# WU-CVGL/CasualHDRSplat

Measured on AMD Instinct MI355X. Metric: train-step images/sec (fwd+bwd raster) @ 1M Gaussians 1080p, higher is better.
Workload: dtype f32; 1 GPU; c3: 1000000 Gaussians, 1920x1080, SH degree 3, HDR radiance + CRF tone-map, 1 pose(s)/view, 1 view(s)/step (one per GPU); num_rendered_R=6777809, R_prime=3025699, pixel_pair_evals_E=559372855, seed=0, binning=sync-free fixed capacity 1.25*R, launch=eager (one enqueue per kernel)

## Files before the change

### casualhdrsplat_amd/csrc/hs_common.h

```cpp
#pragma once
#include <hip/hip_runtime.h>
#include <stdint.h>

#include "../../include/hdrsplat.h"

#if defined(__HIP_DEVICE_COMPILE__) && !defined(__gfx950__)
#error "libhdrsplat is written for gfx950 (MI355X) only: build with --offload-arch=gfx950"
#endif

namespace hs {

void set_error(const char* fmt, ...);

#define HS_HIP_CHECK(expr)                                                                         \
    do {                                                                                           \
        hipError_t e_ = (expr);                                                                    \
        if (e_ != hipSuccess) {                                                                    \
            ::hs::set_error("%s failed: %s (%s:%d)", #expr, hipGetErrorString(e_), __FILE__, __LINE__); \
            return HS_EHIP;                                                                        \
        }                                                                                          \
    } while (0)
#define HS_LAUNCH_CHECK() HS_HIP_CHECK(hipGetLastError())

#ifndef HS_TUNE_CRF_IN_RENDER_TAIL
#define HS_TUNE_CRF_IN_RENDER_TAIL 1
#endif

#ifndef HS_TUNE_COUNT_SORT
#define HS_TUNE_COUNT_SORT 1
#endif

constexpr int kTile = HS_TILE;
constexpr int kRecF4 = 4;
constexpr int kPairF4 = 4;
constexpr int kInstF4 = 4;
constexpr int kRecFloats = 4 * kRecF4;
constexpr int kPairFloats = 4 * kPairF4;
constexpr int kInstFloats = 4 * kInstF4;
constexpr int kSortBlock = 256;
constexpr int kDepthBins = 512, kDepthDigitBits = 9;
#ifndef HS_TUNE_DEPTH_ITEMS
#define HS_TUNE_DEPTH_ITEMS 8
#endif
constexpr int kDepthSortItems = HS_TUNE_DEPTH_ITEMS, kDepthSortLook = 8;
constexpr int kPairSortItems = 16, kPairSortLook = 8;
constexpr int kU64SortItems = 16;
constexpr int kDepthTile = kDepthSortItems * kDepthBins, kPairTile = kPairSortItems * kSortBlock, kU64Tile = kU64SortItems * kSortBlock;
static_assert(kPairTile == kU64Tile && kDepthTile >= kPairTile, "the scratch of every sort is sized for the smallest tile");
constexpr int kSortTileMin = kPairTile;

static inline int64_t align_up(int64_t v, int64_t a) { return (v + a - 1) / a * a; }
static inline int ceil_div(int64_t a, int64_t b) { return (int)((a + b - 1) / b); }

static inline int tile_bits(uint32_t n) {
    int b = 0;
    while (n) { ++b; n >>= 1; }
    return b;
}

int launch_preprocess_fwd(const hs_fwd_args& a, const hs_layout& L, hipStream_t s, uint32_t frame_tag);
int launch_scan(const hs_fwd_args& a, const hs_layout& L, hipStream_t s);
int launch_cov3d(const hs_fwd_args& a, const hs_layout& L, hipStream_t s);
int launch_binning(const hs_fwd_args& a, const hs_layout& L, hipStream_t s, uint32_t frame_tag);
int launch_empty_frame(hs_counters* clear, uint2* ranges, int64_t ntiles, uint32_t* counters_host, const hs_counters* counters,
                       hipStream_t s);
int launch_render_fwd(const hs_fwd_args& a, const hs_layout& L, hipStream_t s, unsigned long long* stats = nullptr);
int launch_render_bwd(const hs_bwd_args& a, const hs_layout& L, hipStream_t s, unsigned long long* stats = nullptr,
                      unsigned long long* timeline = nullptr, bool crf_in_tail = false);
int render_stats_count();
struct CrfReduce;
int launch_crf_bwd(const hs_bwd_args& a, const hs_layout& L, hipStream_t s, CrfReduce* defer, bool in_render_tail = false);
int launch_preprocess_bwd(const hs_bwd_args& a, const hs_layout& L, hipStream_t s, bool segsum, bool project,
                          const CrfReduce* crf_reduce);
int launch_mark_visible(int P, const float* means3D, const float* view, uint8_t* vis, hipStream_t s);
int launch_spline_poses(int J, int T, int kind, const float* delta, const float* base, const float* times, float* w2c,
                        float* jac, int* seg, hipStream_t s);
int launch_sh_backward_views(int P, int M, int deg, int V, const float* means3D, const float* camposes,
                             const float* view_colors, float* d_shs, hipStream_t s);

constexpr int kGhistCopies = 16;
constexpr int kGhistWords = kGhistCopies * 8 * 256;
constexpr int kTicketWords = 128, kDepthBitsAt = 32, kDepthBitsCopies = 16, kDepthBitsWords = 4 * kDepthBitsCopies;
static_assert(kDepthBitsAt >= 8 && kDepthBitsAt % 2 == 0 && kDepthBitsAt + kDepthBitsWords <= kTicketWords, "depth bits live in the ticket row");
__host__ __device__ inline int64_t sweep_pass_words(int64_t nblk, int bins = 256) { return nblk * bins; }
static inline int64_t sort_scratch_words(int64_t n, int passes, int tile, int bins = 256) {
    return n > 0 ? kGhistWords + kTicketWords + (int64_t)passes * sweep_pass_words((n + tile - 1) / tile, bins) : 0;
}
static inline int64_t depth_scratch_words(int64_t I) { return sort_scratch_words(I, 4, kDepthTile, kDepthBins); }
int64_t sort_tmp_bytes(int64_t n);
constexpr int kMsdBits = 12, kMsdBuckets = 1 << kMsdBits;
#ifndef HS_TUNE_MSD_RANGE
// ... 226 lines not shown
```

### casualhdrsplat_amd/csrc/preprocess.hip

```cpp
#include "hs_common.h"


namespace hs {

namespace {

__device__ constexpr float SH_C0 = 0.28209479177387814f;
__device__ constexpr float SH_C1 = 0.4886025119029199f;
__device__ constexpr float SH_C2[5] = {1.0925484305920792f, -1.0925484305920792f, 0.31539156525252005f,
                                       -1.0925484305920792f, 0.5462742152960396f};
__device__ constexpr float SH_C3[7] = {-0.5900435899266435f, 2.890611442640554f, -0.4570457994644658f,
                                       0.3731763325901154f,  -0.4570457994644658f, 1.445305721320277f,
                                       -0.5900435899266435f};

struct Ewa {
    float tx, ty, tz;
    bool clamp_x, clamp_y;
    float a0[3], a1[3];
    float fx, fy;
};

__device__ __forceinline__ void quat_to_R(const float* q, float* R) {
    float r = q[0], x = q[1], y = q[2], z = q[3];
    R[0] = 1.f - 2.f * (y * y + z * z); R[1] = 2.f * (x * y - r * z);       R[2] = 2.f * (x * z + r * y);
// ... 94 lines not shown
            g[14][0] = SH_C3[5] * 2.f * x * z; g[14][1] = SH_C3[5] * -2.f * y * z; g[14][2] = SH_C3[5] * (xx - yy);
            g[15][0] = SH_C3[6] * (3.f * xx - 3.f * yy); g[15][1] = SH_C3[6] * -6.f * x * y;
        }
    }
}

struct PreFwd {
    int P, M, W, H, N;
    float tanfovx, tanfovy, mod;
    const float* view; const float* proj; const float* campos;
    const float* means; const float* opac; const float* shs; const float* colors; const float* scales;
    const float* rots; const float* cov_pre;
    float4* rec; float* depth; int* radii_inst; uint32_t* tiles; float* cov3D; uint8_t* clamped;
    uint2* binfo;
    int* radii_out;
    uint2* depth_pairs; hs_counters* counters; uint2* ranges; int64_t n_vtiles;
    uint32_t* sort_zero; int64_t n_sort_zero;
    int64_t bits_at;
    uint32_t frame_tag;
    uint32_t* pair_zero; int64_t n_pair_zero;
    bool antialias;
    int act;
};

#ifndef HS_TUNE_PF_REC_LDS
#define HS_TUNE_PF_REC_LDS 1
#endif
#ifndef HS_TUNE_PF_EARLY
#define HS_TUNE_PF_EARLY 1
#endif
#ifndef HS_TUNE_PF_WAVES
#define HS_TUNE_PF_WAVES 5
#endif
#if HS_TUNE_PF_WAVES > 0
#define HS_PF_OCC __attribute__((amdgpu_waves_per_eu(HS_TUNE_PF_WAVES, HS_TUNE_PF_WAVES)))
#else
#define HS_PF_OCC
#endif
template <int DEG>
__global__ void __launch_bounds__(256) HS_PF_OCC preprocess_fwd_kernel(PreFwd p) {
    __shared__ uint32_t s_two[2];
    if (p.depth_pairs) {
        if (threadIdx.x < 2) s_two[threadIdx.x] = 0u;
        __syncthreads();
    }
    uint32_t depth_key = 0xFFFFFFFFu;
    const int64_t lin = (int64_t)blockIdx.x * 256 + threadIdx.x;
    const int xcd = blockIdx.x & 7, seq = blockIdx.x >> 3;
    const int pose = seq % p.N;
    const int64_t g64 = ((int64_t)(seq / p.N) * 8 + xcd) * 256 + threadIdx.x;
    uint32_t ntiles = 0;
#if HS_TUNE_PF_REC_LDS
    __shared__ float4 s_rec[4][64 * 4];
    float4 rec_a = make_float4(0.f, 0.f, 0.f, 0.f), rec_b = rec_a, rec_c = rec_a;
#endif
    if (g64 < (int64_t)p.P) {
    const int g = (int)g64;
    const int64_t idx = (int64_t)pose * p.P + g;
    const float* V = p.view + 16 * pose;
    const float* PM = p.proj + 16 * pose;

    int my_radius = 0;
    uint2 bi = make_uint2(0u, 0u);
    float4 ra = make_float4(0.f, 0.f, 0.f, 0.f), rb = ra, rc = ra;
    float depth = 0.f;
    uint8_t clampbits = 0;

    const float x = p.means[3 * g], y = p.means[3 * g + 1], z = p.means[3 * g + 2];
    float sc[3] = {0.f, 0.f, 0.f};
    float4 q4 = make_float4(0.f, 0.f, 0.f, 0.f);
    float s6[6] = {0.f, 0.f, 0.f, 0.f, 0.f, 0.f};
    if (p.cov_pre) {
#pragma unroll
        for (int k = 0; k < 6; ++k) s6[k] = p.cov_pre[6 * g + k];
    } else {
        sc[0] = p.scales[3 * g]; sc[1] = p.scales[3 * g + 1]; sc[2] = p.scales[3 * g + 2];
        q4 = reinterpret_cast<const float4*>(p.rots)[g];
    }
    const float opac_in = p.opac[g];
    const float pvx = xform_row(V, 0, x, y, z), pvy = xform_row(V, 1, x, y, z), pvz = xform_row(V, 2, x, y, z);
    const float phx = xform_row(PM, 0, x, y, z), phy = xform_row(PM, 1, x, y, z), phw = xform_row(PM, 3, x, y, z);
    const float pw = 1.0f / (phw + 0.0000001f);
    const float ppx = phx * pw, ppy = phy * pw;
    constexpr int NCF = (DEG + 1) * (DEG + 1);
    float shr[3 * NCF];
#pragma unroll
    for (int k = 0; k < 3 * NCF; ++k) shr[k] = 0.f;
    bool have_sh = false;
    bool vis = false;
#if HS_TUNE_PF_EARLY
    const bool early = !p.colors && pvz > 0.2f && fabsf(ppx) < 1.5f && fabsf(ppy) < 1.5f;
    if (early) {
        const float* sh = p.shs + (int64_t)g * p.M * 3;
#pragma unroll
        for (int k = 0; k < 3 * NCF; ++k) shr[k] = sh[k];
        have_sh = true;
    }
#endif
    if (!p.cov_pre && (pose == 0 || pvz > 0.2f)) {
        float q[4] = {q4.x, q4.y, q4.z, q4.w};
        cov3d_from_scale_rot(sc, p.mod, q, s6);
    }

    if (pvz > 0.2f) {

        Ewa e;
        ewa_setup(V, p.W, p.H, p.tanfovx, p.tanfovy, pvx, pvy, pvz, e);
        float u0[3], u1[3];
        sym_mul(s6, e.a0, u0);
        sym_mul(s6, e.a1, u1);
        const float ca = dot3(e.a0, u0) + 0.3f;
        const float cb = dot3(e.a1, u0);
        const float cc = dot3(e.a1, u1) + 0.3f;
        const float det = ca * cc - cb * cb;
        if (det != 0.0f) {
            const float det_inv = 1.f / det;
            const float conA = cc * det_inv, conB = -cb * det_inv, conC = ca * det_inv;
            const float mid = 0.5f * (ca + cc);
            const float disc = sqrtf(fmaxf(0.1f, mid * mid - det));
            const float lam1 = mid + disc, lam2 = mid - disc;
            const int rad = (int)ceilf(3.f * sqrtf(fmaxf(lam1, lam2)));
            const float pix_x = ((ppx + 1.0f) * (float)p.W - 1.0f) * 0.5f;
            const float pix_y = ((ppy + 1.0f) * (float)p.H - 1.0f) * 0.5f;
            const int gx = (p.W + kTile - 1) / kTile, gy = (p.H + kTile - 1) / kTile;
            const int rminx = min(gx, max(0, (int)((pix_x - (float)rad) / (float)kTile)));
            const int rminy = min(gy, max(0, (int)((pix_y - (float)rad) / (float)kTile)));
            const int rmaxx = min(gx, max(0, (int)((pix_x + (float)rad + (float)(kTile - 1)) / (float)kTile)));
            const int rmaxy = min(gy, max(0, (int)((pix_y + (float)rad + (float)(kTile - 1)) / (float)kTile)));
            const int area = (rmaxx - rminx) * (rmaxy - rminy);
            if (area != 0) {
                vis = true;
                my_radius = rad;
                ntiles = (uint32_t)area;
                bi = make_uint2((uint32_t)rminx | ((uint32_t)rminy << 16),
                                (uint32_t)(rmaxx - rminx) | ((uint32_t)(rmaxy - rminy) << 16));
                depth = pvz;
                ra = make_float4(pix_x, pix_y, conA, conB);
                float opac = opac_in;
                if (p.antialias) {
                    const float det0 = (ca - 0.3f) * (cc - 0.3f) - cb * cb;
                    opac = opac * sqrtf(fmaxf(0.000025f, det0 / det));
                }
                rb = make_float4(conC, opac, 0.f, 0.f);
                rc = make_float4(0.f, pvz, __int_as_float(rad), 0.f);
            }
        }
    }
    if (vis) {
        float col[3];
        if (p.colors) {
            col[0] = p.colors[3 * g]; col[1] = p.colors[3 * g + 1]; col[2] = p.colors[3 * g + 2];
        } else {
            const float* cp = p.campos + 3 * pose;
            const float dx = x - cp[0], dy = y - cp[1], dz = z - cp[2];
            const float len = sqrtf((dx * dx + dy * dy) + dz * dz);
            const float ux = dx / len, uy = dy / len, uz = dz / len;
            float b[(DEG + 1) * (DEG + 1)];
            sh_basis<DEG>(ux, uy, uz, b);
            if (!have_sh) {
                const float* sh = p.shs + (int64_t)g * p.M * 3;
#pragma unroll
                for (int k = 0; k < 3 * NCF; ++k) shr[k] = sh[k];
            }
            float acc[3] = {b[0] * shr[0], b[0] * shr[1], b[0] * shr[2]};
#pragma unroll
            for (int k = 1; k < (DEG + 1) * (DEG + 1); ++k) {
                acc[0] = acc[0] + b[k] * shr[3 * k + 0];
                acc[1] = acc[1] + b[k] * shr[3 * k + 1];
                acc[2] = acc[2] + b[k] * shr[3 * k + 2];
            }
#pragma unroll
            for (int ch = 0; ch < 3; ++ch) {
                if (p.act == 1) {
                    col[ch] = expf(acc[ch]);
                } else if (p.act == 2) {
                    col[ch] = acc[ch] > 20.f ? acc[ch] : log1pf(expf(acc[ch]));
                } else {
                    float v = acc[ch] + 0.5f;
                    if (v < 0.f) clampbits |= (uint8_t)(1u << ch);
                    col[ch] = fmaxf(v, 0.f);
                }
            }
        }
        rb.z = col[0]; rb.w = col[1]; rc.x = col[2];
    }
#if HS_TUNE_PF_REC_LDS
    rec_a = ra; rec_b = rb; rec_c = rc;
#else
    p.rec[kRecF4 * idx + 0] = ra;
    p.rec[kRecF4 * idx + 1] = rb;
    p.rec[kRecF4 * idx + 2] = rc;
    p.rec[kRecF4 * idx + 3] = make_float4(0.f, 0.f, 0.f, 0.f);
#endif
    p.depth[idx] = depth;
    p.radii_inst[idx] = my_radius;
    p.tiles[idx] = ntiles;
    p.binfo[idx] = bi;
    p.clamped[idx] = clampbits;
    if (p.N == 1) p.radii_out[g] = my_radius;
    else if (my_radius > 0) atomicMax(p.radii_out + g, my_radius);
    if (p.depth_pairs) {
        if (my_radius > 0) depth_key = __float_as_uint(depth);
        p.depth_pairs[idx] = make_uint2(depth_key, (uint32_t)idx);
    }
    }
#if HS_TUNE_PF_REC_LDS
    {
        const int lane = threadIdx.x & 63, wave = threadIdx.x >> 6;
        float4* w = s_rec[wave];
        const int sw = (lane >> 2) & 3;
        w[lane * 4 + (0 ^ sw)] = rec_a;
        w[lane * 4 + (1 ^ sw)] = rec_b;
        w[lane * 4 + (2 ^ sw)] = rec_c;
        w[lane * 4 + (3 ^ sw)] = make_float4(0.f, 0.f, 0.f, 0.f);
        __builtin_amdgcn_fence(__ATOMIC_RELEASE, "wavefront");
        __builtin_amdgcn_wave_barrier();
        const int64_t g_w0 = g64 - lane;
        const int nvalid = (int)min((int64_t)64, (int64_t)p.P - g_w0);
        float4* dst = p.rec + kRecF4 * ((int64_t)pose * p.P + g_w0);
#pragma unroll
        for (int j = 0; j < 4; ++j) {
            const int f = j * 64 + lane, r = f >> 2, k = f & 3;
            if (r < nvalid) dst[f] = w[r * 4 + (k ^ ((r >> 2) & 3))];
        }
    }
#endif
    if (p.depth_pairs) {
        depth_bits_accumulate(depth_key, depth_key != 0xFFFFFFFFu,
                              reinterpret_cast<unsigned long long*>(p.sort_zero + p.bits_at), p.frame_tag, s_two);
        for (int64_t t = lin; t < p.n_vtiles; t += (int64_t)gridDim.x * 256) p.ranges[t] = make_uint2(0u, 0u);
        for (int64_t t = lin; t < p.n_sort_zero; t += (int64_t)gridDim.x * 256)
            if (t < p.bits_at || t >= p.bits_at + kDepthBitsWords) p.sort_zero[t] = 0u;
        for (int64_t t = lin; t < p.n_pair_zero; t += (int64_t)gridDim.x * 256) p.pair_zero[t] = 0u;
        if (lin == 0) {
            p.counters->overflow = 0u;
            p.counters->reserved[1] = (uint32_t)((int64_t)p.P * p.N);
            p.counters->reserved[2] = 0u; p.counters->reserved[3] = 0u;
            p.counters->reserved[4] = 0u;
        }
    }
}

__global__ void __launch_bounds__(256) cov3d_kernel(int P, float mod, const float* scales, const float* rots, const float* cov_pre,
                                                    float* cov3D) {
    const int g = blockIdx.x * 256 + threadIdx.x;
    if (g >= P) return;
    float s6[6];
    if (cov_pre) {
#pragma unroll
        for (int k = 0; k < 6; ++k) s6[k] = cov_pre[6 * (int64_t)g + k];
    } else {
        float sc[3] = {scales[3 * g], scales[3 * g + 1], scales[3 * g + 2]};
        const float4 q4 = reinterpret_cast<const float4*>(rots)[g];
        float q[4] = {q4.x, q4.y, q4.z, q4.w};
        cov3d_from_scale_rot(sc, mod, q, s6);
    }
#pragma unroll
    for (int k = 0; k < 6; ++k) cov3D[6 * (int64_t)g + k] = s6[k];
}

__global__ void mark_visible_kernel(int P, const float* means, const float* V, uint8_t* vis) {
    int i = blockIdx.x * 256 + threadIdx.x;
    if (i >= P) return;
    vis[i] = xform_row(V, 2, means[3 * i], means[3 * i + 1], means[3 * i + 2]) > 0.2f;
}

__global__ void __launch_bounds__(256) pair_segsum_kernel(SegsumArgs sg, CrfReduce crf_reduce) {
// ... 639 lines not shown
```

### casualhdrsplat_amd/csrc/render.hip

```cpp
#include "hs_common.h"

namespace hs {

namespace {

constexpr float kAlphaMin = 1.0f / 255.0f;
constexpr float kAlphaMax = 0.99f;
constexpr float kTmin = 0.0001f;
constexpr float kLogEps = 1e-8f;


enum {
    kStBwdTrips = 0,
    kStBwdEmpty = 1,
    kStBwdActivePix = 2,
    kStBwdCulled = 3,
    kStBwdHist = 4,
    kStBwdStaged = 10,
    kStBwdBatches = 11,
    kStFwdTrips = 12, kStFwdEmpty = 13, kStFwdActivePix = 14, kStFwdCulled = 15, kStFwdStaged = 16, kStFwdBatches = 17,
    kStCount = 24
};
struct WaveStats {
    unsigned long long v[kStCount];
    __device__ __forceinline__ void clear() {
#pragma unroll
        for (int i = 0; i < kStCount; ++i) v[i] = 0;
    }
    __device__ __forceinline__ void flush(unsigned long long* dst) const {
        if ((threadIdx.x & 63) == 0) {
#pragma unroll
            for (int i = 0; i < kStCount; ++i)
                if (v[i]) atomicAdd(dst + i, v[i]);
        }
    }
};

template <int CTRL, int ROW_MASK = 0xF>
__device__ __forceinline__ float dpp(float v) {
    return __int_as_float(__builtin_amdgcn_update_dpp(0, __float_as_int(v), CTRL, ROW_MASK, 0xF, false));
}
__device__ __forceinline__ float wave_sum_hi(float v) {
    v += dpp<0xB1>(v);
    v += dpp<0x4E>(v);
    v += dpp<0x141>(v);
    v += dpp<0x140>(v);
    v += dpp<0x142, 0xA>(v);
    v += dpp<0x143, 0xC>(v);
    return v;
}
__device__ __forceinline__ float halve16(float x, float y) {
    auto r = __builtin_amdgcn_permlane16_swap(__float_as_uint(x), __float_as_uint(y), false, false);
    return __uint_as_float(r[0]) + __uint_as_float(r[1]);
}
template <bool TEN>
__device__ __forceinline__ void reduce_in_rows(const float* g, float g9, float& w0, float& w1, float& w2) {
    float z0, z1, z2, z3, z4;
    if constexpr (TEN) {
        asm("s_nop 1\n\t"
// ... 49 lines not shown
template <bool TEN>
__device__ __forceinline__ void group_reduce(const float* g, float g9, int xor16_addr, float& t0, float& t1) {
    float w0, w1, w2;
    reduce_in_rows<TEN>(g, g9, w0, w1, w2);
    const float u0 = halve16(w0, w1);
    const float u1 = w2 + __int_as_float(__builtin_amdgcn_ds_bpermute(xor16_addr, __float_as_int(w2)));
    t0 = reduce_in_quads(u0);
    t1 = reduce_in_quads(u1);
}

__device__ __forceinline__ int mask_prefix(uint64_t m) {
    return (int)__builtin_amdgcn_mbcnt_hi((uint32_t)(m >> 32), __builtin_amdgcn_mbcnt_lo((uint32_t)m, 0u));
}

__device__ __forceinline__ uint32_t wave_max_u32(uint32_t v) {
#pragma unroll
    for (int d = 32; d >= 1; d >>= 1) v = max(v, (uint32_t)__shfl_xor((int)v, d));
    return v;
}

struct Crf {
    const float* table;
    int K;
    float umin, umax, dt;
};

__device__ __forceinline__ void crf_locate(const Crf& c, float Hv, int& i, float& f, float& xv, bool& interior) {
    xv = Hv * c.dt;
    const float u = __logf(fmaxf(xv, kLogEps));
    float s = (u - c.umin) / (c.umax - c.umin) * (float)(c.K - 1);
    bool in = true;
    if (!(s > 0.f)) { s = 0.f; in = false; }
    if (s >= (float)(c.K - 1)) { s = (float)(c.K - 1); in = false; }
    i = (int)floorf(s);
    if (i > c.K - 2) i = c.K - 2;
    f = s - (float)i;
    interior = in && (xv > kLogEps);
}
__device__ __forceinline__ float crf_eval(const Crf& c, int ch, float Hv) {
    int i; float f, xv; bool in;
    crf_locate(c, Hv, i, f, xv, in);
    const float* t = c.table + ch * c.K;
    return t[i] * (1.f - f) + t[i + 1] * f;
}
__device__ __forceinline__ float crf_grad_H(const Crf& c, int ch, float Hv, float g) {
    int i; float f, xv; bool in;
    crf_locate(c, Hv, i, f, xv, in);
    if (!in) return 0.f;
    const float* t = c.table + ch * c.K;
    const float scale = (float)(c.K - 1) / (c.umax - c.umin);
    return g * (t[i + 1] - t[i]) * scale / xv * c.dt;
}

constexpr float kLog2e = 1.4426950408889634f;

typedef float f2 __attribute__((ext_vector_type(2)));

#ifndef HS_NO_OPSEL_ASM
__device__ __forceinline__ f2 pk_fma_hi(f2 pair, f2 w, f2 acc) {
    asm("v_pk_fma_f32 %0, %1, %2, %0 op_sel:[1,0,0] op_sel_hi:[1,1,1]" : "+v"(acc) : "v"(pair), "v"(w));
    return acc;
}
__device__ __forceinline__ f2 pk_mul_hi(f2 pair, f2 w) {
    f2 r;
    asm("v_pk_mul_f32 %0, %1, %2 op_sel:[1,0] op_sel_hi:[1,1]" : "=v"(r) : "v"(pair), "v"(w));
    return r;
}
#else
__device__ __forceinline__ f2 pk_fma_hi(f2 pair, f2 w, f2 acc) { return acc + f2{pair.y, pair.y} * w; }
__device__ __forceinline__ f2 pk_mul_hi(f2 pair, f2 w) { return f2{pair.y, pair.y} * w; }
#endif

__device__ __forceinline__ void scale_entry(float4& a, float4& b) {
    a.z *= -0.5f * kLog2e; a.w *= -kLog2e; b.x *= -0.5f * kLog2e;
}

template <int WIDTH>
__device__ __forceinline__ bool block_may_touch(const float4 a, const float4 b, float sx, float sy) {
    const float A2 = a.z, B2 = a.w, C2 = b.x, o = b.y;
    if (!(o >= kAlphaMin)) return false;
    if (!(A2 < 0.f && C2 < 0.f && 4.f * A2 * C2 - B2 * B2 > 0.f)) return true;
    const float thr = -(__log2f(255.f * o) * 1.0001f + 0.05f);
    const float dx_lo = a.x - (sx + (float)(WIDTH - 1)), dx_hi = a.x - sx, dy_lo = a.y - (sy + 7.f), dy_hi = a.y - sy;
    const float dx_e = fminf(fmaxf(0.f, dx_lo), dx_hi);
    const float dy_e = fminf(fmaxf(0.f, dy_lo), dy_hi);
    const float dy_s = fminf(fmaxf(-0.5f * B2 * dx_e / C2, dy_lo), dy_hi);
    const float dx_s = fminf(fmaxf(-0.5f * B2 * dy_e / A2, dx_lo), dx_hi);
    const float p1 = dx_e * (A2 * dx_e + B2 * dy_s) + C2 * dy_s * dy_s;
    const float p2 = dx_s * (A2 * dx_s + B2 * dy_e) + C2 * dy_e * dy_e;
    return fmaxf(p1, p2) >= thr;
}

__device__ __forceinline__ void lane_pixels(int lane, int sx, int sy, int& px, int& py0) {
    px = sx + 8 * (lane >> 5) + (lane & 7);
    py0 = sy + 2 * ((lane >> 3) & 3);
}

struct RenderFwd {
    int W, H, gx, ntiles, N, flags;
    const uint2* ranges; const uint32_t* point_list; const float4* rec; const float* bg;
    float* out_color; float* out_hdr; float* final_T; uint32_t* n_contrib; float* pose_hdr;
    float* out_invdepth;
    Crf crf;
    const float* exposure;
    unsigned long long* stats;
    unsigned long long* timeline;
    uint8_t* pair_act;
    uint32_t* tile_work;
};

constexpr int kBatch = 128;

__device__ __forceinline__ int xcd_strip_tile(int b, int nb, int gx) {
    constexpr int kXcd = 8, kRows = 2;
    const int x = b % kXcd, k = b / kXcd;
    const int per = nb / kXcd, rem = nb % kXcd;
    int p = x * per + min(x, rem) + k;
    const int rows = nb / gx;
    const int nstrips = (rows + kRows - 1) / kRows;
    const int strip_tiles = kRows * gx;
    const int last_short = nstrips * strip_tiles - nb;
    int c = 0;
    for (; c < kXcd - 1; ++c) {
        const int ns = (nstrips - c + kXcd - 1) / kXcd;
        const int nt = ns * strip_tiles - (((nstrips - 1) % kXcd) == c ? last_short : 0);
        if (p < nt) break;
        p -= nt;
    }
    const int s_local = p / strip_tiles, r = p - s_local * strip_tiles;
    return (c + kXcd * s_local) * strip_tiles + r;
}

__device__ __forceinline__ float hs_exp2(float x) { return __builtin_amdgcn_exp2f(x); }

struct PixF {
    float T, C0, C1, C2, D;
    uint32_t last;
};
constexpr int kFcmpOGE = 3, kFcmpOLE = 5;
struct PairF {
    f2 T, C0, C1, C2, D;
    uint32_t last0, last1;
};
// ... 11 lines not shown
    done0 |= valid0 ^ cont0;
    done1 |= valid1 ^ cont1;
    const bool upd0 = __builtin_amdgcn_inverse_ballot_w64(cont0), upd1 = __builtin_amdgcn_inverse_ballot_w64(cont1);
    const f2 aT = alpha * s.T;
    const f2 w = {upd0 ? aT.x : 0.f, upd1 ? aT.y : 0.f};
    const f2 rr = {r, r}, bb = {b, b};
    s.C0 += rr * w; s.C1 = pk_fma_hi(f2{r, g}, w, s.C1); s.C2 += bb * w;
    if constexpr (DEPTH) { const f2 dd = {invd, invd}; s.D += dd * w; }
    s.T = f2{upd0 ? test_T.x : s.T.x, upd1 ? test_T.y : s.T.y};
    s.last0 = upd0 ? idx1 : s.last0;
    s.last1 = upd1 ? idx1 : s.last1;
    if (n_pixels) *n_pixels = __popcll(cont0) + __popcll(cont1);
    return cont0 | cont1;
}

__device__ __forceinline__ void write_pixel_fwd(const RenderFwd& p, const PixF& st, int pose, int px, int py) {
    const int64_t HW = (int64_t)p.H * p.W;
    const int64_t pix = (int64_t)py * p.W + px;
    p.final_T[(int64_t)pose * HW + pix] = st.T;
    p.n_contrib[(int64_t)pose * HW + pix] = st.last;
    const float H0 = st.C0 + st.T * p.bg[0], H1 = st.C1 + st.T * p.bg[1], H2 = st.C2 + st.T * p.bg[2];
    const bool hdr = p.flags & HS_FLAG_HDR;
    if (p.pose_hdr) {
        float* ph = p.pose_hdr + (int64_t)pose * 3 * HW;
        ph[pix] = H0; ph[HW + pix] = H1; ph[2 * HW + pix] = H2;
    }
    if (p.N == 1) {
        if (hdr) {
            Crf c = p.crf;
            c.dt = p.exposure[0];
            if (p.out_hdr) { p.out_hdr[pix] = H0; p.out_hdr[HW + pix] = H1; p.out_hdr[2 * HW + pix] = H2; }
            p.out_color[pix] = crf_eval(c, 0, H0);
            p.out_color[HW + pix] = crf_eval(c, 1, H1);
            p.out_color[2 * HW + pix] = crf_eval(c, 2, H2);
        } else {
            p.out_color[pix] = H0; p.out_color[HW + pix] = H1; p.out_color[2 * HW + pix] = H2;
        }
    }
}

constexpr int kFwdEntF = 12;

template <bool DEPTH, bool STATS>
__global__ void __launch_bounds__(kBatch) __attribute__((amdgpu_waves_per_eu((DEPTH || STATS) ? 1 : 7)))
render_fwd_kernel(RenderFwd p) {
    constexpr int KB = kBatch;
    constexpr int kEnt = kFwdEntF * 4;
    constexpr int kSentinel = KB * kEnt;
    constexpr int kListLen = KB + 8;
    __shared__ __attribute__((aligned(16))) float s_ent[(KB + 1) * kFwdEntF];
    __shared__ int s_alive[2][2];
    __shared__ uint16_t s_list[2][2][kListLen];
    __shared__ uint8_t s_taken[2][2][KB];
    __shared__ uint32_t s_work[2];

    const int vt = xcd_strip_tile(blockIdx.x, gridDim.x, p.gx);
    const int pose = vt / p.ntiles;
    const int tile = vt - pose * p.ntiles;
    const int tx = tile % p.gx, ty = tile / p.gx;
    const int wave = threadIdx.x >> 6, lane = threadIdx.x & 63;
    const int grp = lane >> 5;
    const int sx = tx * kTile, sy = ty * kTile + wave * 8;
    int px, py0;
    lane_pixels(lane, sx, sy, px, py0);
    const int py1 = py0 + 1;
    const bool in0 = px < p.W && py0 < p.H, in1 = px < p.W && py1 < p.H;
    const float pxf = (float)px;
    const f2 pyf = {(float)py0, (float)py1};
    const float sxf = (float)sx, syf = (float)sy;

    const uint2 range = p.ranges[vt];
    const int n = (int)(range.y - range.x);

    PairF ps;
    ps.T = f2{1.f, 1.f};
    ps.C0 = ps.C1 = ps.C2 = ps.D = f2{0.f, 0.f};
    ps.last0 = ps.last1 = 0;
    uint64_t done0 = __builtin_amdgcn_ballot_w64(!in0), done1 = __builtin_amdgcn_ballot_w64(!in1);

    float4 ra = make_float4(0.f, 0.f, 0.f, 0.f), rb = ra;
    float rcb = 0.f, rdepth = 1.f;
    if ((int)threadIdx.x < n) {
        const uint32_t id = p.point_list[range.x + threadIdx.x];
        const float4* r = p.rec + kRecF4 * (int64_t)id;
        ra = r[0]; rb = r[1]; rcb = reinterpret_cast<const float*>(r + 2)[0];
        if constexpr (DEPTH) rdepth = reinterpret_cast<const float*>(r + 2)[1];
    }
    WaveStats ws;
    if constexpr (STATS) ws.clear();
    const char* const ent = reinterpret_cast<const char*>(s_ent);
    float* const my_ent = s_ent + threadIdx.x * kFwdEntF;
    const uint16_t* const my_list = s_list[wave][grp];
    if (threadIdx.x < kFwdEntF) s_ent[KB * kFwdEntF + threadIdx.x] = 0.f;
    auto flush_activity = [&](int base_prev, int cnt_prev) {
        const int t = threadIdx.x;
        if (t < cnt_prev)
            p.pair_act[(int64_t)range.x + base_prev + t] = (uint8_t)(s_taken[0][0][t] | s_taken[0][1][t] | s_taken[1][0][t] | s_taken[1][1][t]);
        s_taken[0][0][t] = 0; s_taken[0][1][t] = 0; s_taken[1][0][t] = 0; s_taken[1][1][t] = 0;
    };
    auto walk = [&](int i0, int i1, int base48) -> uint32_t {
        uint32_t act_lo = 0u, act_hi = 0u;
        uint32_t pos = 0u;
        const uint32_t npos = (uint32_t)(i1 - i0);
        const uint16_t* lp = my_list + i0;
        auto trip = [&]() {
            const int jb = (int)*lp++;
            const char* e = ent + jb;
            const float4 a = *reinterpret_cast<const float4*>(e);
            const float4 b = *reinterpret_cast<const float4*>(e + 16);
            const float2 c = *reinterpret_cast<const float2*>(e + 32);
            const float dx = a.x - pxf;
            const f2 dy = a.y - pyf;
            const float t = a.z * dx * dx, u = a.w * dx;
            const f2 pw = dy * (b.x * dy + u) + t;
            const float al0 = fminf(kAlphaMax, b.y * hs_exp2(pw.x));
            const float al1 = fminf(kAlphaMax, b.y * hs_exp2(pw.y));
            const uint32_t idx48 = (uint32_t)(base48 + jb + kEnt);
            int n_pix = 0;
            const uint64_t took = blend_fwd_pair<DEPTH>(ps, done0, done1, pw, f2{al0, al1}, b.z, b.w, c.x, DEPTH ? c.y : 0.f, idx48,
                                                        STATS ? &n_pix : nullptr);
            if constexpr (STATS) ws.v[kStFwdActivePix] += n_pix;
#pragma clang diagnostic push
#pragma clang diagnostic ignored "-Winline-asm"
            asm("s_mov_b32 m0, %2\n\t"
                "v_writelane_b32 %0, %3, m0\n\t"
                "v_writelane_b32 %1, %4, m0\n\t"
                "s_add_u32 %2, %2, 1"
                : "+v"(act_lo), "+v"(act_hi), "+s"(pos) : "s"((uint32_t)took), "s"((uint32_t)(took >> 32)) : "scc", "m0");
#pragma clang diagnostic pop
            if constexpr (STATS) { ws.v[kStFwdTrips] += 1; ws.v[kStFwdEmpty] += took == 0ull; }
        };
        if (npos >= 2u) {
            do {
                trip();
                trip();
            } while (pos + 2u <= npos && (done0 & done1) != ~0ull);
        }
        if (pos + 1u == npos && (done0 & done1) != ~0ull) trip();
        return (act_lo != 0u ? 1u : 0u) | (act_hi != 0u ? 4u : 0u);
    };
    s_taken[0][0][threadIdx.x] = 0; s_taken[0][1][threadIdx.x] = 0; s_taken[1][0][threadIdx.x] = 0; s_taken[1][1][threadIdx.x] = 0;
    uint32_t n_taken = 0;
    int it = 0, base = 0;
    for (; base < n; base += KB, ++it) {
        const uint64_t fin = done0 & done1;
        const bool wave_alive = fin != ~0ull;
        if (lane == 0) s_alive[it & 1][wave] = wave_alive;
        __syncthreads();
        if (it > 0) flush_activity(base - KB, KB);
        if (!(s_alive[it & 1][0] | s_alive[it & 1][1])) break;
        const int cnt = min(KB, n - base);
        if constexpr (STATS) { if (wave == 0) { ws.v[kStFwdStaged] += cnt; ws.v[kStFwdBatches] += 1; } }
        if ((int)threadIdx.x < cnt) {
            scale_entry(ra, rb);
            reinterpret_cast<float4*>(my_ent)[0] = ra;
            reinterpret_cast<float4*>(my_ent)[1] = rb;
            reinterpret_cast<float2*>(my_ent)[4] = make_float2(rcb, DEPTH ? 1.f / rdepth : 0.f);
        }
        if (base + KB + (int)threadIdx.x < n) {
            const uint32_t id = p.point_list[range.x + base + KB + threadIdx.x];
            const float4* r = p.rec + kRecF4 * (int64_t)id;
            ra = r[0]; rb = r[1]; rcb = reinterpret_cast<const float*>(r + 2)[0];
            if constexpr (DEPTH) rdepth = reinterpret_cast<const float*>(r + 2)[1];
        }
        __syncthreads();
        if (wave_alive) {
            const bool alive_g[2] = {(uint32_t)fin != 0xFFFFFFFFu, (uint32_t)(fin >> 32) != 0xFFFFFFFFu};
            int n_g[2] = {0, 0};
#pragma unroll
            for (int k = 0; k < KB / 64; ++k) {
                const int jj = k * 64 + lane;
                bool touch[2] = {false, false};
                if (jj < cnt) {
                    const float4 a = reinterpret_cast<const float4*>(s_ent + jj * kFwdEntF)[0];
                    const float4 b = reinterpret_cast<const float4*>(s_ent + jj * kFwdEntF)[1];
                    touch[0] = alive_g[0] && block_may_touch<8>(a, b, sxf, syf);
                    touch[1] = alive_g[1] && block_may_touch<8>(a, b, sxf + 8.f, syf);
                }
                if constexpr (STATS) ws.v[kStFwdCulled] += __popcll(__ballot(jj < cnt && !touch[0] && !touch[1]));
#pragma unroll
                for (int g = 0; g < 2; ++g) {
                    const uint64_t mask = __ballot(touch[g]);
                    if (touch[g]) s_list[wave][g][n_g[g] + mask_prefix(mask)] = (uint16_t)(jj * kEnt);
                    n_g[g] += __popcll(mask);
                }
            }
            const int n_t = max(n_g[0], n_g[1]);
#pragma unroll
            for (int g = 0; g < 2; ++g)
#pragma unroll
                for (int t = lane; t < kListLen; t += 64)
                    if (t >= n_g[g]) s_list[wave][g][t] = (uint16_t)kSentinel;
            const uint32_t t0 = walk(0, min(n_t, 64), base * kEnt);
            const uint32_t t1 = ((done0 & done1) != ~0ull && n_t > 64) ? walk(64, n_t, base * kEnt) : 0u;

#pragma unroll
            for (int g = 0; g < 2; ++g) {
                const uint32_t bit = 1u << (2 * g);
                if (t0 & bit) s_taken[wave][g][s_list[wave][g][lane] / kEnt] = (uint8_t)(bit << wave);
                if (t1 & bit) s_taken[wave][g][s_list[wave][g][64 + lane] / kEnt] = (uint8_t)(bit << wave);
                n_taken += (uint32_t)(__popcll(__ballot((t0 & bit) != 0u)) + __popcll(__ballot((t1 & bit) != 0u)));
            }
        }
    }
    if (it > 0 && base >= n) {
        __syncthreads();
        flush_activity(base - KB, n - (base - KB));
    }
    if (lane == 0) s_work[wave] = n_taken;
    __syncthreads();
    if (threadIdx.x == 0) p.tile_work[vt] = s_work[0] + s_work[1];
    {
        float* const o = s_ent + wave * (6 * 128);
        const int pos0 = (py0 - sy) * 16 + (px - sx), pos1 = pos0 + 16;
        o[pos0] = ps.T.x; o[pos1] = ps.T.y;
        o[128 + pos0] = __uint_as_float(ps.last0); o[128 + pos1] = __uint_as_float(ps.last1);
        o[256 + pos0] = ps.C0.x; o[256 + pos1] = ps.C0.y;
        o[384 + pos0] = ps.C1.x; o[384 + pos1] = ps.C1.y;
        o[512 + pos0] = ps.C2.x; o[512 + pos1] = ps.C2.y;
        if constexpr (DEPTH) { o[640 + pos0] = ps.D.x; o[640 + pos1] = ps.D.y; }
        const int qx = sx + (lane & 15), qy0 = sy + 2 * (lane >> 4);
        const int r0 = (qy0 - sy) * 16 + (lane & 15), r1 = r0 + 16;
        PixF s0, s1;
        s0.T = o[r0]; s0.last = __float_as_uint(o[128 + r0]) / (kFwdEntF * 4); s0.C0 = o[256 + r0]; s0.C1 = o[384 + r0]; s0.C2 = o[512 + r0];
        s1.T = o[r1]; s1.last = __float_as_uint(o[128 + r1]) / (kFwdEntF * 4); s1.C0 = o[256 + r1]; s1.C1 = o[384 + r1]; s1.C2 = o[512 + r1];
        const bool q0 = qx < p.W && qy0 < p.H, q1 = qx < p.W && qy0 + 1 < p.H;
        if (q0) write_pixel_fwd(p, s0, pose, qx, qy0);
        if (q1) write_pixel_fwd(p, s1, pose, qx, qy0 + 1);
        if constexpr (DEPTH) {
            const int64_t HW = (int64_t)p.H * p.W;
            if (q0) p.out_invdepth[(int64_t)pose * HW + (int64_t)qy0 * p.W + qx] = o[640 + r0];
            if (q1) p.out_invdepth[(int64_t)pose * HW + (int64_t)(qy0 + 1) * p.W + qx] = o[640 + r1];
        }
    }
    if constexpr (STATS) ws.flush(p.stats);
}

__global__ void __launch_bounds__(256) resolve_kernel(int64_t HW, int N, int flags, float* pose_hdr, Crf crf,
                                                      const float* exposure, float* out_color, float* out_hdr) {
    const int64_t i = (int64_t)blockIdx.x * 256 + threadIdx.x;
    if (i >= 3 * HW) return;
    const int ch = (int)(i / HW);
    const bool hdr = flags & HS_FLAG_HDR;
    if (hdr) crf.dt = exposure[0];
    float sumH = 0.f, sumL = 0.f;
    for (int k = 0; k < N; ++k) {
        const float Hv = pose_hdr[(int64_t)k * 3 * HW + i];
        sumH += Hv;
        if (hdr && !(flags & HS_FLAG_BLUR_HDR)) sumL += crf_eval(crf, ch, Hv);
    }
    const float inv = 1.f / (float)N;
    const float meanH = sumH * inv;
    pose_hdr[(int64_t)N * 3 * HW + i] = meanH;
    if (hdr) {
        if (out_hdr) out_hdr[i] = meanH;
        out_color[i] = (flags & HS_FLAG_BLUR_HDR) ? crf_eval(crf, ch, meanH) : sumL * inv;
    } else {
        out_color[i] = meanH;
    }
}

__global__ void __launch_bounds__(1024) order_tiles_kernel(int nb, int gx, int n_static, const uint32_t* work,
                                                           uint32_t* order) {
    constexpr int kBins = 1024, kT = 1024;
    __shared__ uint32_t s_hist[kBins];
    __shared__ uint32_t s_scan[kT / 64];
    __shared__ uint32_t s_thr_bin, s_thr_take, s_cnt_thr, s_cnt_q;
    const int x = blockIdx.x, t = threadIdx.x;
    const int per = nb / 8, rem = nb % 8;
    const int cnt = per + (x < rem ? 1 : 0);
    const int n_keep = n_static > x ? (n_static - x + 7) / 8 : 0;
    const int n_light = cnt - n_keep;
    int q_base = 0;
    for (int y = 0; y < x; ++y) q_base += (per + (y < rem ? 1 : 0)) - (n_static > y ? (n_static - y + 7) / 8 : 0);
    const int E = (cnt + kT - 1) / kT;
// ... 627 lines not shown
```

Before: 965.6 images/s.

## Precompute per-Gaussian cull constants in preprocess; cull 8x8 blocks once per tile

Preprocess now writes the fourth record float4 (previously zero) with a cull threshold and the conic-axis slopes, using a double-precision definiteness test. In the forward render, each staged Gaussian is tested once per thread against all four 8x8 sub-blocks of the 16x16 tile, producing a bitmask in LDS. The two waves then read that mask instead of each re-running the block_may_touch test with its divisions and log. The record's fourth float4 is now loaded per entry, adding some bandwidth, and the output-pixel LDS indexing is rewritten to a lane-derived formula.

```diff
diff --git a/casualhdrsplat_amd/csrc/hs_common.h b/casualhdrsplat_amd/csrc/hs_common.h
--- a/casualhdrsplat_amd/csrc/hs_common.h
+++ b/casualhdrsplat_amd/csrc/hs_common.h
@@ -37,6 +37,21 @@
 constexpr int kRecFloats = 4 * kRecF4;
 constexpr int kPairFloats = 4 * kPairF4;
 constexpr int kInstFloats = 4 * kInstF4;
+
+constexpr float kAlphaMin = 1.0f / 255.0f;
+constexpr float kLog2e = 1.4426950408889634f;
+
+__device__ __forceinline__ float4 rec_cull(float conA, float conB, float conC, float o) {
+    const float inf = __builtin_inff();
+    if (!(o >= kAlphaMin)) return make_float4(inf, 0.f, 0.f, 0.f);
+    const float A2 = conA * (-0.5f * kLog2e), B2 = conB * -kLog2e, C2 = conC * (-0.5f * kLog2e);
+    const double d4ac = 4.0 * (double)A2 * (double)C2, dbb = (double)B2 * (double)B2;
+    const float ky = (-0.5f * B2) / C2, kx = (-0.5f * B2) / A2;
+    const bool definite = A2 < 0.f && C2 < 0.f && d4ac - dbb > 0x1p-20 * d4ac &&
+                          fabsf(ky) <= 3.0e38f && fabsf(kx) <= 3.0e38f;
+    if (!definite) return make_float4(-inf, 0.f, 0.f, 0.f);
+    return make_float4(-fmaf(__log2f(255.f * o), 1.0001f, 0.05f), ky, kx, 0.f);
+}
 constexpr int kSortBlock = 256;
 constexpr int kDepthBins = 512, kDepthDigitBits = 9;
 #ifndef HS_TUNE_DEPTH_ITEMS
diff --git a/casualhdrsplat_amd/csrc/preprocess.hip b/casualhdrsplat_amd/csrc/preprocess.hip
--- a/casualhdrsplat_amd/csrc/preprocess.hip
+++ b/casualhdrsplat_amd/csrc/preprocess.hip
@@ -170,7 +170,7 @@
     uint32_t ntiles = 0;
 #if HS_TUNE_PF_REC_LDS
     __shared__ float4 s_rec[4][64 * 4];
-    float4 rec_a = make_float4(0.f, 0.f, 0.f, 0.f), rec_b = rec_a, rec_c = rec_a;
+    float4 rec_a = make_float4(0.f, 0.f, 0.f, 0.f), rec_b = rec_a, rec_c = rec_a, rec_d = rec_a;
 #endif
     if (g64 < (int64_t)p.P) {
     const int g = (int)g64;
@@ -180,7 +180,7 @@
 
     int my_radius = 0;
     uint2 bi = make_uint2(0u, 0u);
-    float4 ra = make_float4(0.f, 0.f, 0.f, 0.f), rb = ra, rc = ra;
+    float4 ra = make_float4(0.f, 0.f, 0.f, 0.f), rb = ra, rc = ra, rd = ra;
     float depth = 0.f;
     uint8_t clampbits = 0;
 
@@ -260,6 +260,7 @@
                     opac = opac * sqrtf(fmaxf(0.000025f, det0 / det));
                 }
                 rb = make_float4(conC, opac, 0.f, 0.f);
+                rd = rec_cull(conA, conB, conC, opac);
                 rc = make_float4(0.f, pvz, __int_as_float(rad), 0.f);
             }
         }
@@ -303,12 +304,12 @@
         rb.z = col[0]; rb.w = col[1]; rc.x = col[2];
     }
 #if HS_TUNE_PF_REC_LDS
-    rec_a = ra; rec_b = rb; rec_c = rc;
+    rec_a = ra; rec_b = rb; rec_c = rc; rec_d = rd;
 #else
     p.rec[kRecF4 * idx + 0] = ra;
     p.rec[kRecF4 * idx + 1] = rb;
     p.rec[kRecF4 * idx + 2] = rc;
-    p.rec[kRecF4 * idx + 3] = make_float4(0.f, 0.f, 0.f, 0.f);
+    p.rec[kRecF4 * idx + 3] = rd;
 #endif
     p.depth[idx] = depth;
     p.radii_inst[idx] = my_radius;
@@ -330,7 +331,7 @@
         w[lane * 4 + (0 ^ sw)] = rec_a;
         w[lane * 4 + (1 ^ sw)] = rec_b;
         w[lane * 4 + (2 ^ sw)] = rec_c;
-        w[lane * 4 + (3 ^ sw)] = make_float4(0.f, 0.f, 0.f, 0.f);
+        w[lane * 4 + (3 ^ sw)] = rec_d;
         __builtin_amdgcn_fence(__ATOMIC_RELEASE, "wavefront");
         __builtin_amdgcn_wave_barrier();
         const int64_t g_w0 = g64 - lane;
diff --git a/casualhdrsplat_amd/csrc/render.hip b/casualhdrsplat_amd/csrc/render.hip
--- a/casualhdrsplat_amd/csrc/render.hip
+++ b/casualhdrsplat_amd/csrc/render.hip
@@ -4,7 +4,6 @@
 
 namespace {
 
-constexpr float kAlphaMin = 1.0f / 255.0f;
 constexpr float kAlphaMax = 0.99f;
 constexpr float kTmin = 0.0001f;
 constexpr float kLogEps = 1e-8f;
@@ -160,8 +159,6 @@
     return g * (t[i + 1] - t[i]) * scale / xv * c.dt;
 }
 
-constexpr float kLog2e = 1.4426950408889634f;
-
 typedef float f2 __attribute__((ext_vector_type(2)));
 
 #ifndef HS_NO_OPSEL_ASM
@@ -183,20 +180,39 @@
     a.z *= -0.5f * kLog2e; a.w *= -kLog2e; b.x *= -0.5f * kLog2e;
 }
 
-template <int WIDTH>
-__device__ __forceinline__ bool block_may_touch(const float4 a, const float4 b, float sx, float sy) {
-    const float A2 = a.z, B2 = a.w, C2 = b.x, o = b.y;
-    if (!(o >= kAlphaMin)) return false;
-    if (!(A2 < 0.f && C2 < 0.f && 4.f * A2 * C2 - B2 * B2 > 0.f)) return true;
-    const float thr = -(__log2f(255.f * o) * 1.0001f + 0.05f);
-    const float dx_lo = a.x - (sx + (float)(WIDTH - 1)), dx_hi = a.x - sx, dy_lo = a.y - (sy + 7.f), dy_hi = a.y - sy;
-    const float dx_e = fminf(fmaxf(0.f, dx_lo), dx_hi);
-    const float dy_e = fminf(fmaxf(0.f, dy_lo), dy_hi);
-    const float dy_s = fminf(fmaxf(-0.5f * B2 * dx_e / C2, dy_lo), dy_hi);
-    const float dx_s = fminf(fmaxf(-0.5f * B2 * dy_e / A2, dx_lo), dx_hi);
-    const float p1 = dx_e * (A2 * dx_e + B2 * dy_s) + C2 * dy_s * dy_s;
-    const float p2 = dx_s * (A2 * dx_s + B2 * dy_e) + C2 * dy_e * dy_e;
-    return fmaxf(p1, p2) >= thr;
+#ifndef HS_TUNE_FWD_CULL
+#define HS_TUNE_FWD_CULL 1
+#endif
+
+__device__ __forceinline__ float clampf(float v, float lo, float hi) { return __builtin_amdgcn_fmed3f(v, lo, hi); }
+
+__device__ __forceinline__ uint32_t tile_block_mask(const float4 a, float C2, const float4 q, float tx0, float ty0) {
+    const float A2 = a.z, B2 = a.w;
+    float dx_lo[2], dx_hi[2], dx_e[2], dy_v[2], dy_lo[2], dy_hi[2], dy_e[2], dx_v[2];
+#pragma unroll
+    for (int c = 0; c < 2; ++c) {
+        dx_lo[c] = a.x - (tx0 + (float)(8 * c + 7)); dx_hi[c] = a.x - (tx0 + (float)(8 * c));
+        dx_e[c] = clampf(0.f, dx_lo[c], dx_hi[c]);
+        dy_v[c] = q.y * dx_e[c];
+    }
+#pragma unroll
+    for (int r = 0; r < 2; ++r) {
+        dy_lo[r] = a.y - (ty0 + (float)(8 * r + 7)); dy_hi[r] = a.y - (ty0 + (float)(8 * r));
+        dy_e[r] = clampf(0.f, dy_lo[r], dy_hi[r]);
+        dx_v[r] = q.z * dy_e[r];
+    }
+    uint32_t m = 0u;
+#pragma unroll
+    for (int r = 0; r < 2; ++r)
+#pragma unroll
+        for (int c = 0; c < 2; ++c) {
+            const float dy_s = clampf(dy_v[c], dy_lo[r], dy_hi[r]);
+            const float dx_s = clampf(dx_v[r], dx_lo[c], dx_hi[c]);
+            const float p1 = dx_e[c] * (A2 * dx_e[c] + B2 * dy_s) + C2 * dy_s * dy_s;
+            const float p2 = dx_s * (A2 * dx_s + B2 * dy_e[r]) + C2 * dy_e[r] * dy_e[r];
+            if (!(fmaxf(p1, p2) < q.x)) m |= 1u << (2 * r + c);
+        }
+    return m;
 }
 
 __device__ __forceinline__ void lane_pixels(int lane, int sx, int sy, int& px, int& py0) {
@@ -314,6 +330,7 @@
     __shared__ int s_alive[2][2];
     __shared__ uint16_t s_list[2][2][kListLen];
     __shared__ uint8_t s_taken[2][2][KB];
+    __shared__ uint8_t s_blocks[KB];
     __shared__ uint32_t s_work[2];
 
     const int vt = xcd_strip_tile(blockIdx.x, gridDim.x, p.gx);
@@ -329,7 +346,7 @@
     const bool in0 = px < p.W && py0 < p.H, in1 = px < p.W && py1 < p.H;
     const float pxf = (float)px;
     const f2 pyf = {(float)py0, (float)py1};
-    const float sxf = (float)sx, syf = (float)sy;
+    const float txf = (float)(tx * kTile), tyf = (float)(ty * kTile);
 
     const uint2 range = p.ranges[vt];
     const int n = (int)(range.y - range.x);
@@ -340,13 +357,14 @@
     ps.last0 = ps.last1 = 0;
     uint64_t done0 = __builtin_amdgcn_ballot_w64(!in0), done1 = __builtin_amdgcn_ballot_w64(!in1);
 
-    float4 ra = make_float4(0.f, 0.f, 0.f, 0.f), rb = ra;
+    float4 ra = make_float4(0.f, 0.f, 0.f, 0.f), rb = ra, rq = ra;
     float rcb = 0.f, rdepth = 1.f;
     if ((int)threadIdx.x < n) {
         const uint32_t id = p.point_list[range.x + threadIdx.x];
         const float4* r = p.rec + kRecF4 * (int64_t)id;
         ra = r[0]; rb = r[1]; rcb = reinterpret_cast<const float*>(r + 2)[0];
         if constexpr (DEPTH) rdepth = reinterpret_cast<const float*>(r + 2)[1];
+        if (HS_TUNE_FWD_CULL) rq = r[3];
     }
     WaveStats ws;
     if constexpr (STATS) ws.clear();
@@ -413,17 +431,21 @@
         if (!(s_alive[it & 1][0] | s_alive[it & 1][1])) break;
         const int cnt = min(KB, n - base);
         if constexpr (STATS) { if (wave == 0) { ws.v[kStFwdStaged] += cnt; ws.v[kStFwdBatches] += 1; } }
+        uint32_t blocks = 0u;
         if ((int)threadIdx.x < cnt) {
             scale_entry(ra, rb);
             reinterpret_cast<float4*>(my_ent)[0] = ra;
             reinterpret_cast<float4*>(my_ent)[1] = rb;
             reinterpret_cast<float2*>(my_ent)[4] = make_float2(rcb, DEPTH ? 1.f / rdepth : 0.f);
-        }
+            blocks = HS_TUNE_FWD_CULL ? tile_block_mask(ra, rb.x, rq, txf, tyf) : 0xFu;
+        }
+        s_blocks[threadIdx.x] = (uint8_t)blocks;
         if (base + KB + (int)threadIdx.x < n) {
             const uint32_t id = p.point_list[range.x + base + KB + threadIdx.x];
             const float4* r = p.rec + kRecF4 * (int64_t)id;
             ra = r[0]; rb = r[1]; rcb = reinterpret_cast<const float*>(r + 2)[0];
             if constexpr (DEPTH) rdepth = reinterpret_cast<const float*>(r + 2)[1];
+            if (HS_TUNE_FWD_CULL) rq = r[3];
         }
         __syncthreads();
         if (wave_alive) {
@@ -432,13 +454,8 @@
 #pragma unroll
             for (int k = 0; k < KB / 64; ++k) {
                 const int jj = k * 64 + lane;
-                bool touch[2] = {false, false};
-                if (jj < cnt) {
-                    const float4 a = reinterpret_cast<const float4*>(s_ent + jj * kFwdEntF)[0];
-                    const float4 b = reinterpret_cast<const float4*>(s_ent + jj * kFwdEntF)[1];
-                    touch[0] = alive_g[0] && block_may_touch<8>(a, b, sxf, syf);
-                    touch[1] = alive_g[1] && block_may_touch<8>(a, b, sxf + 8.f, syf);
-                }
+                const uint32_t bl = (uint32_t)s_blocks[jj] >> (2 * wave);
+                const bool touch[2] = {alive_g[0] && (bl & 1u) != 0u, alive_g[1] && (bl & 2u) != 0u};
                 if constexpr (STATS) ws.v[kStFwdCulled] += __popcll(__ballot(jj < cnt && !touch[0] && !touch[1]));
 #pragma unroll
                 for (int g = 0; g < 2; ++g) {
@@ -474,15 +491,17 @@
     if (threadIdx.x == 0) p.tile_work[vt] = s_work[0] + s_work[1];
     {
         float* const o = s_ent + wave * (6 * 128);
-        const int pos0 = (py0 - sy) * 16 + (px - sx), pos1 = pos0 + 16;
+        int ln = lane;
+        asm volatile("" : "+v"(ln));
+        const int pos0 = ((ln >> 3) & 3) * 32 + (ln >> 5) * 8 + (ln & 7), pos1 = pos0 + 16;
         o[pos0] = ps.T.x; o[pos1] = ps.T.y;
         o[128 + pos0] = __uint_as_float(ps.last0); o[128 + pos1] = __uint_as_float(ps.last1);
         o[256 + pos0] = ps.C0.x; o[256 + pos1] = ps.C0.y;
         o[384 + pos0] = ps.C1.x; o[384 + pos1] = ps.C1.y;
         o[512 + pos0] = ps.C2.x; o[512 + pos1] = ps.C2.y;
         if constexpr (DEPTH) { o[640 + pos0] = ps.D.x; o[640 + pos1] = ps.D.y; }
-        const int qx = sx + (lane & 15), qy0 = sy + 2 * (lane >> 4);
-        const int r0 = (qy0 - sy) * 16 + (lane & 15), r1 = r0 + 16;
+        const int qx = sx + (ln & 15), qy0 = sy + 2 * (ln >> 4);
+        const int r0 = (qy0 - sy) * 16 + (ln & 15), r1 = r0 + 16;
         PixF s0, s1;
         s0.T = o[r0]; s0.last = __float_as_uint(o[128 + r0]) / (kFwdEntF * 4); s0.C0 = o[256 + r0]; s0.C1 = o[384 + r0]; s0.C2 = o[512 + r0];
         s1.T = o[r1]; s1.last = __float_as_uint(o[128 + r1]) / (kFwdEntF * 4); s1.C0 = o[256 + r1]; s1.C1 = o[384 + r1]; s1.C2 = o[512 + r1];
```

Result: faster. 978.4 images/s (median of 6 runs) (+1.3%).
